# wkentaro/chainer-mask-rcnn

Measured on AMD Instinct MI355X. Metric: images/sec train step, ResNet50-C4 Mask R-CNN, COCO 800x1333, higher is better.
Workload: dtype f32 (bf16x3 split operands, f32 accumulate)

## Files before the change

chainer_mask_rcnn_amd/csrc/conv_gemm.hip:

```cpp
#include <algorithm>
#include <cstring>

#include "conv_gemm_kernel.h"

namespace {

__global__ void splitk_reduce_kernel(const float *__restrict__ ws, int splits, int64_t n,
                                     int64_t stride, float *__restrict__ out)
{
    const int64_t nv = n / 4;
    for (int64_t i = (int64_t)blockIdx.x * blockDim.x + threadIdx.x; i < nv;
         i += (int64_t)gridDim.x * blockDim.x) {
        float4 a = reinterpret_cast<const float4 *>(ws)[i];
        int s = 1;
        for (; s + 4 <= splits; s += 4) {
            const float4 v0 = reinterpret_cast<const float4 *>(ws + (s + 0) * stride)[i];
            const float4 v1 = reinterpret_cast<const float4 *>(ws + (s + 1) * stride)[i];
            const float4 v2 = reinterpret_cast<const float4 *>(ws + (s + 2) * stride)[i];
            const float4 v3 = reinterpret_cast<const float4 *>(ws + (s + 3) * stride)[i];
            a.x += v0.x; a.y += v0.y; a.z += v0.z; a.w += v0.w;
            a.x += v1.x; a.y += v1.y; a.z += v1.z; a.w += v1.w;
            a.x += v2.x; a.y += v2.y; a.z += v2.z; a.w += v2.w;
            a.x += v3.x; a.y += v3.y; a.z += v3.z; a.w += v3.w;
        }
        for (; s < splits; ++s) {
            const float4 v = reinterpret_cast<const float4 *>(ws + s * stride)[i];
            a.x += v.x; a.y += v.y; a.z += v.z; a.w += v.w;
        }
        reinterpret_cast<float4 *>(out)[i] = a;
    }
}

GemmKnobs g_knobs;

inline GemmShape gemm_shape(const GemmParams &p, int mode, bool has_ws)
{
    GemmShape g = {};
    g.mode = mode;
    g.M = p.M; g.N = p.N; g.Kc = p.Kc;
    g.R = p.R; g.S = p.S; g.stride = p.stride; g.pad = p.pad;
    g.gp = p.gp; g.gq = p.gq; g.sh = p.sh; g.sw = p.sw;
    g.ldc = p.ldc; g.out_mode = p.out_mode; g.stem = p.stem; g.perm_n = p.perm_n;
    g.has_ws = has_ws;
    return g;
}

template <int TM, int TN, int MODE>
void launch_kernel(const GemmParams &p, GemmInst inst, int64_t tiles, int splits, hipStream_t s, int batch = 1)
{
    hipEvent_t ev0, ev1;
    mrcnn::prof_take(&ev0, &ev1);
    auto go = [&](auto kernel) {
        hipExtLaunchKernelGGL(kernel, dim3((unsigned)tiles, splits, batch), dim3(256), 0, s, ev0, ev1, 0, p);
    };
    if constexpr (TM == TN && ((MODE == WGRAD && TM == 2) || (MODE == FWD && (TM == 1 || TM == 2)))) {
        if (inst.split) {
            const dim3 grid((unsigned)tiles, splits, batch);
            if (inst.planes == 1) return launch_planes<1>(p, 64 * TM, MODE, inst.variant, grid, s, ev0, ev1);
            if (inst.planes == 2) return launch_planes<2>(p, 64 * TM, MODE, inst.variant, grid, s, ev0, ev1);
            if constexpr (MODE == FWD) {
                if (inst.variant == INST_PW) return go(conv_gemm_kernel<TM, TN, MODE, false, 3, false, true>);
                if (inst.variant == INST_K3) return go(conv_gemm_kernel<TM, TN, MODE, false, 3, false, false, true>);
            }
            return go(conv_gemm_kernel<TM, TN, MODE, false, 3>);
        }
    }
    if constexpr (MODE == WGRAD) {
        if (inst.variant == INST_WPERM) return go(conv_gemm_kernel<TM, TN, MODE, true>);
    }
    go(conv_gemm_kernel<TM, TN, MODE>);
}

template <int TM, int TN, int MODE>
void launch_wino_kernel(const GemmParams &p, const GemmLaunch &l, hipStream_t s)
{
    launch_kernel<TM, TN, MODE>(p, l.inst, l.grid_x, l.grid_y, s, kWinoXi);
}

void launch_w8_kernel(const GemmParams &p, int64_t wgs, int batch, hipStream_t s, int planes = 3)
{
    hipEvent_t ev0, ev1;
    mrcnn::prof_take(&ev0, &ev1);
    const dim3 grid((unsigned)wgs, 1, batch);
    if (planes == 1) return launch_planes<1>(p, kW8BM, FWD, INST_W8, grid, s, ev0, ev1);
    if (planes == 2) return launch_planes<2>(p, kW8BM, FWD, INST_W8, grid, s, ev0, ev1);
    hipExtLaunchKernelGGL((conv_gemm_kernel<2, 2, FWD, false, 3, true>), grid, dim3(512), 0, s, ev0, ev1, 0, p);
}

template <int MODE>
mrcnn::ProfKernelScope gemm_prof(const GemmParams &p, const GemmLaunch &l)
{
    const int small = l.tile >= 128 ? 0 : 1;
    if (MODE == WGRAD)
        return mrcnn::ProfKernelScope(mrcnn::PROF_CONV_WGRAD_128 + small, 2.0 * p.M * p.N * (double)p.Kc,
                                      4.0 * ((double)p.M * p.N + (double)p.Kc * (p.M + (double)p.cin)));
    const int64_t rows = l.m_hi - l.m_lo;
    const double kdepth = (double)p.R * p.S * (p.stem ? 21.0 : (double)p.Kc);
    const double flops = 2.0 * rows * p.N * kdepth;
    const double bytes = 4.0 * ((double)rows * p.N + (double)rows * p.Kc + (double)p.N * kdepth);
    const int kind = l.tile == kW8BM ? mrcnn::PROF_CONV_FWD_W8
                                     : (MODE == FWD ? mrcnn::PROF_CONV_FWD_128 : mrcnn::PROF_CONV_DGRAD_128) + small;
    return mrcnn::ProfKernelScope(kind, flops, bytes);
}

struct FixParams {
    const float *ws;
    float *C;
    const float *bias, *scale, *shift, *residual, *res_g, *res_y, *out_mask_y;
    int splits, rows, N, row0, ldc, flags;
    int perm_n, pq;
    int64_t stride;
};

__global__ void __launch_bounds__(256) splitk_epilogue_kernel(const FixParams f)
{
    const int n4 = f.N / 4;
    const int64_t i = (int64_t)blockIdx.x * blockDim.x + threadIdx.x;
    if (i >= (int64_t)f.rows * n4) return;
    const int r = (int)(i / n4), c = (int)(i - (int64_t)r * n4) * 4;
    float4 a = *reinterpret_cast<const float4 *>(f.ws + (int64_t)r * f.N + c);
    for (int s = 1; s < f.splits; ++s) {
        const float4 v = *reinterpret_cast<const float4 *>(f.ws + s * f.stride + (int64_t)r * f.N + c);
        a.x += v.x; a.y += v.y; a.z += v.z; a.w += v.w;
    }
    float v[4] = {a.x, a.y, a.z, a.w};
    int orow = f.row0 + r;
    if (f.perm_n > 0) {
        const PermRow pr = perm_row(orow, f.pq);
        if (pr.n >= f.perm_n) return;
        orow = pr.n * f.pq + pr.pos;
    }
    const int64_t off = (int64_t)orow * f.ldc + c;
#pragma unroll
    for (int k = 0; k < 4; ++k) {
        float x = v[k];
        if (f.flags & MRCNN_EPI_BIAS) x += f.bias[c + k];
        if (f.flags & MRCNN_EPI_AFFINE) x = x * f.scale[c + k] + (f.shift ? f.shift[c + k] : 0.f);
        if (f.flags & MRCNN_EPI_RESIDUAL) x += f.residual[off + k];
        if (f.flags & MRCNN_EPI_ACCUM) x += f.C[off + k];
        if (f.res_g) x += (!f.res_y || f.res_y[off + k] > 0.f) ? f.res_g[off + k] : 0.f;
        if (f.flags & MRCNN_EPI_RELU) x = fmaxf(x, 0.f);
        if (f.out_mask_y) x = f.out_mask_y[off + k] > 0.f ? x : 0.f;
        v[k] = x;
    }
    *reinterpret_cast<float4 *>(f.C + off) = make_float4(v[0], v[1], v[2], v[3]);
}

template <int MODE>
void slab_sum(const GemmParams &p, int rows_lo, int splits, hipStream_t s)
{
    const int rows = p.M - rows_lo;
    FixParams f = {};
    f.ws = p.split_ws; f.C = p.C;
    f.bias = p.bias; f.scale = p.scale; f.shift = p.shift; f.residual = p.residual;
    f.res_g = p.res_g; f.res_y = p.res_y; f.out_mask_y = p.out_mask_y;
    f.splits = splits; f.rows = rows; f.N = p.N; f.row0 = rows_lo; f.ldc = p.ldc;
    f.flags = p.flags; f.stride = (int64_t)rows * p.N;
    f.perm_n = MODE == FWD ? p.perm_n : 0; f.pq = p.gp * p.gq;
    const int64_t n = (int64_t)rows * (p.N / 4);
    hipLaunchKernelGGL(splitk_epilogue_kernel, dim3((unsigned)mrcnn::ceil_div(n, 256)), dim3(256), 0, s, f);
}

template <int MODE>
int run_plan(const GemmParams &p, const GemmPlan &plan, hipStream_t s)
{
    for (int i = 0; i < plan.n; ++i) {
        const GemmLaunch &l = plan.launch[i];
        GemmParams q = p;
        q.m_lo = l.m_lo;
        q.M = l.m_hi;
        if constexpr (MODE == WGRAD) {
            q.perm_n = plan.perm_n;
            q.split_len = l.split_len;
            q.split_stride = (int64_t)p.M * p.N;
            q.C = plan.sum_splits ? p.split_ws : p.C;
            q.split_ws = nullptr;
        } else if (l.split_len) {
            q.C = p.split_ws;
            q.flags = 0;
            q.bias = q.scale = q.shift = q.residual = q.res_g = q.res_y = q.out_mask_y = nullptr;
            q.split_len = l.split_len;
            q.split_stride = (int64_t)(l.m_hi - l.m_lo) * p.N;
            q.out_row0 = l.m_lo;
            q.c_bytes = (unsigned)(q.split_stride * 4);
        }
        if (l.tail_splits) {
            q.tail_first = l.tail_first;
            q.tail_row0 = l.tail_row0;
            q.tail_splits = l.tail_splits;
            q.tail_split_len = l.tail_split_len;
            q.tail_ws = p.split_ws;
            q.tail_stride = (int64_t)(l.m_hi - l.tail_row0) * p.N;
            q.tail_bytes = (unsigned)(q.tail_stride * 4);
        }
        const auto prof = gemm_prof<MODE>(p, l);
        if (l.tile == kW8BM) {
            if constexpr (MODE == FWD) launch_w8_kernel(q, l.grid_x, 1, s, l.inst.planes);
        } else if (l.tile == 128) {
            launch_kernel<2, 2, MODE>(q, l.inst, l.grid_x, l.grid_y, s);
        } else {
            launch_kernel<1, 1, MODE>(q, l.inst, l.grid_x, l.grid_y, s);
        }
    }
    if constexpr (MODE == WGRAD) {
        if (plan.sum_splits) {
            const int64_t gwsz = (int64_t)p.M * p.N;
            const int64_t blocks = mrcnn::ceil_div(gwsz / 4, 256);
            hipLaunchKernelGGL(splitk_reduce_kernel, dim3((unsigned)blocks), dim3(256), 0, s,
                               (const float *)p.split_ws, plan.sum_splits, gwsz, gwsz, p.C);
        }
        return mrcnn::check_launch("conv_wgrad");
    } else {
        if (plan.sum_splits) slab_sum<MODE>(p, plan.sum_row0, plan.sum_splits, s);
        return mrcnn::check_launch("conv_gemm");
    }
}

template <int MODE>
int launch(const GemmParams &p, hipStream_t s)
{
    return run_plan<MODE>(p, plan_gemm(gemm_shape(p, MODE, p.split_ws != nullptr), g_knobs), s);
}

int check_desc(const mrcnn_conv_desc *d)
{
    MRCNN_REQUIRE(d, "conv: null descriptor");
    MRCNN_REQUIRE(d->N > 0 && d->H > 0 && d->W > 0 && d->C > 0 && d->K > 0 && d->R > 0 && d->S > 0 &&
                      d->stride > 0 && d->pad >= 0,
                  "conv: bad descriptor");
    MRCNN_REQUIRE(d->P == (d->H + 2 * d->pad - d->R) / d->stride + 1 &&
                      d->Q == (d->W + 2 * d->pad - d->S) / d->stride + 1,
                  "conv: output size (%d,%d) inconsistent with input (%d,%d) k=%d s=%d p=%d", d->P,
                  d->Q, d->H, d->W, d->R, d->stride, d->pad);
// ... 514 lines not shown
```

chainer_mask_rcnn_amd/csrc/conv_gemm_kernel.h:

```cpp
#pragma once
#include <type_traits>

#include "common.h"
#include "conv_gemm_plan.h"

namespace {

using namespace mrcnn::gemm;

typedef float f32x16 __attribute__((ext_vector_type(16)));

constexpr int min_blocks(int tm, int mode)
{
    if (!single_buffered(tm, mode)) return 1;
    return tm == 4 ? 2 : (tm == 2 ? 3 : 6);
}
constexpr int KPAD = 4;

constexpr bool is_fwd(int m) { return m == FWD; }

}

namespace mrcnn {
namespace gemm {

struct GemmParams {
    const float *A;
    const float *B;
    float *C;
    const float *bias, *scale, *shift, *residual;
    int M, N;
    int m_lo;
    int Kc;
    int gp, gq;
    int sh, sw;
    int R, S, stride, pad;
    int lda;
    int ldb;
    int ldg;
    int cin;
    int ldc;
    int flags;
    int out_mode;
    int oh, ow, ko;
    int ostride;
    int stem;
    int split_len;
    int64_t split_stride;
    int out_row0;
    int perm_n;
    const float *res_g, *res_y, *out_mask_y;
    float *split_ws;
    unsigned a_bytes, b_bytes, c_bytes;
    int tail_first, tail_splits, tail_split_len, tail_row0;
    unsigned tail_bytes;
    float *tail_ws;
    int64_t tail_stride;
    int64_t batch_a, batch_b, batch_c;
};

struct PermRow { int n, pos; };
__host__ __device__ __forceinline__ PermRow perm_row(int m, int pq)
{
    const int q = m / kPermBlock, img = m - q * kPermBlock;
    const int blk = q / pq;
    PermRow r;
    r.pos = q - blk * pq;
    r.n = blk * kPermBlock + img;
    return r;
}

template <int NP>
void launch_planes(const GemmParams &p, int tile, int mode, int variant, dim3 grid, hipStream_t s, hipEvent_t ev0,
                   hipEvent_t ev1);
extern template void launch_planes<1>(const GemmParams &, int, int, int, dim3, hipStream_t, hipEvent_t, hipEvent_t);
extern template void launch_planes<2>(const GemmParams &, int, int, int, dim3, hipStream_t, hipEvent_t, hipEvent_t);

}
}

namespace {

template <int TM, int TN, int MODE>
struct Cfg {
    static constexpr int BM = 64 * TM, BN = 64 * TN;
    static constexpr bool A_KC = (MODE != WGRAD);
    static constexpr bool B_KC = is_fwd(MODE);
    static constexpr int A_FLOATS = A_KC ? BM * (BK + KPAD) : BK * BM;
    static constexpr int B_FLOATS = B_KC ? BN * (BK + KPAD) : BK * BN;
    static constexpr int A_V4 = BM * BK / 4 / 256;
    static constexpr int B_V4 = BN * BK / 4 / 256;
};

typedef unsigned int u32x4 __attribute__((ext_vector_type(4)));
constexpr unsigned kOOB = 0x80000000u;

__device__ __forceinline__ __amdgpu_buffer_rsrc_t make_rsrc(const void *p, unsigned bytes)
{
    return __builtin_amdgcn_make_buffer_rsrc(const_cast<void *>(p), 0, p ? bytes : 0u, 0x00020000);
}
__device__ __forceinline__ float4 bload4(__amdgpu_buffer_rsrc_t r, unsigned off)
{
    const u32x4 v = __builtin_amdgcn_raw_buffer_load_b128(r, off, 0, 0);
    return make_float4(__uint_as_float(v.x), __uint_as_float(v.y), __uint_as_float(v.z),
                       __uint_as_float(v.w));
}
__device__ __forceinline__ float bload1(__amdgpu_buffer_rsrc_t r, unsigned off)
{
    return __uint_as_float(__builtin_amdgcn_raw_buffer_load_b32(r, off, 0, 0));
}
__device__ __forceinline__ void bstore1(__amdgpu_buffer_rsrc_t r, unsigned off, float v)
{
    __builtin_amdgcn_raw_buffer_store_b32(__float_as_uint(v), r, off, 0, 0);
}
__device__ __forceinline__ void bstore4(__amdgpu_buffer_rsrc_t r, unsigned off, float4 v)
{
    u32x4 u;
    u.x = __float_as_uint(v.x); u.y = __float_as_uint(v.y);
    u.z = __float_as_uint(v.z); u.w = __float_as_uint(v.w);
    __builtin_amdgcn_raw_buffer_store_b128(u, r, off, 0, 0);
}
__device__ __forceinline__ void bstore8(__amdgpu_buffer_rsrc_t r, unsigned off, unsigned a, unsigned b)
{
    typedef unsigned int u32x2 __attribute__((ext_vector_type(2)));
    u32x2 u;
    u.x = a; u.y = b;
    __builtin_amdgcn_raw_buffer_store_b64(u, r, off, 0, 0);
}

typedef __bf16 bf16x2 __attribute__((ext_vector_type(2)));
typedef __bf16 bf16x8 __attribute__((ext_vector_type(8)));
typedef float f32x2 __attribute__((ext_vector_type(2)));
__device__ __forceinline__ unsigned pack_bf16(float a, float b)
{
    const f32x2 v = {a, b};
    return __builtin_bit_cast(unsigned, __builtin_convertvector(v, bf16x2));
}
__device__ __forceinline__ float sub_f32(float a, float b)
{
    float r;
    asm("v_sub_f32 %0, %1, %2" : "=v"(r) : "v"(a), "v"(b));
    return r;
}
template <int NP = 3>
__device__ __forceinline__ void split3(float a, float b, unsigned &h, unsigned &m, unsigned &l)
{
    h = pack_bf16(a, b);
    if constexpr (NP >= 2) {
        a = sub_f32(a, __uint_as_float(h << 16));
        b = sub_f32(b, __uint_as_float(h & 0xffff0000u));
        m = pack_bf16(a, b);
    }
    if constexpr (NP >= 3) {
        a = sub_f32(a, __uint_as_float(m << 16));
        b = sub_f32(b, __uint_as_float(m & 0xffff0000u));
        l = pack_bf16(a, b);
    }
}

template <int G, int NM, int NMD, int ND, int I = 0>
__device__ __forceinline__ void sgb_interleave()
{
    if constexpr (I < G) {
        constexpr int m0 = NM * I / G, m1 = NM * (I + 1) / G;
        constexpr int d0 = m0 >= NMD ? ND : ND * m0 / NMD, d1 = m1 >= NMD ? ND : ND * m1 / NMD;
        if constexpr (m1 > m0) __builtin_amdgcn_sched_group_barrier(0x008, m1 - m0, 0);
        __builtin_amdgcn_sched_group_barrier(0x020, 1, 0);
        if constexpr (d1 > d0) __builtin_amdgcn_sched_group_barrier(0x100, d1 - d0, 0);
        sgb_interleave<G, NM, NMD, ND, I + 1>();
    }
}

template <int TM, int TN, int MODE, bool WPERM = false, int NP = 0, bool W8 = false,
          bool PW = false, bool K3 = false>
__global__ void __launch_bounds__(W8 ? 512 : 256,
                                  NP > 0 ? (TM == 2 ? 2 : 4) : min_blocks(TM, MODE))
conv_gemm_kernel(const GemmParams p)
{
    static_assert(NP >= 0 && NP <= 3, "NP: 0 (fp32 MFMA) or 1 .. 3 bf16 planes");
    constexpr bool SPLIT = NP > 0;
    constexpr int NPROD = NP == 3 ? 6 : NP == 2 ? 3 : 1;
    static_assert(!W8 || (SPLIT && MODE == FWD && TM == 2 && TN == 2),
                  "W8: the split-operand forward form on 64x64 wave tiles");
    static_assert(!WPERM || MODE == WGRAD, "WPERM is a WGRAD-only variant");
    static_assert(!PW || MODE == FWD, "PW: forward form only");
    static_assert(!K3 || (MODE == FWD && !W8 && !PW), "K3: forward form only");
    constexpr bool PWC = W8 || PW;
    constexpr bool GEO = PWC || K3;
    const int gR = PWC ? 1 : K3 ? 3 : p.R, gS = PWC ? 1 : K3 ? 3 : p.S;
    const int gStride = GEO ? 1 : p.stride, gPad = PWC ? 0 : K3 ? 1 : p.pad;
    const int gPermN = GEO ? 0 : p.perm_n;
    const bool gStem = !GEO && p.stem;
    constexpr bool ILV = SPLIT && MODE == FWD;
    static_assert(!SPLIT || (BK == 32 && TM == TN &&
                             ((MODE == FWD && (TM == 1 || TM == 2)) || (MODE == WGRAD && !WPERM && TM == 2))),
                  "SPLIT: forward form (128x128, 64x64) / weight gradient (128x128) only");
    constexpr bool SINGLEBUF = !W8 && (SPLIT || single_buffered(TM, MODE));
    using C_ = Cfg<TM, TN, MODE>;
    constexpr int NT = W8 ? 512 : 256;
    constexpr int BM = (W8 ? 2 : 1) * C_::BM, BN = C_::BN;
    constexpr int AV = BM * BK / 4 / NT, BV = BN * BK / 4 / NT;
    constexpr bool FWDLIKE = is_fwd(MODE);
    constexpr int SROW = MODE == WGRAD ? BK + 8 : BK;
    constexpr int PLA = BM * SROW, PLB = BN * SROW;
    constexpr int STAGE_FLOATS = SPLIT ? 3 * (PLA + PLB) / 2 : C_::A_FLOATS + C_::B_FLOATS;
    __shared__ __attribute__((aligned(16))) float smem_all[1][SINGLEBUF ? 1 : 2][STAGE_FLOATS];

    float (*smem)[STAGE_FLOATS] = smem_all[0];
    constexpr bool WROWPERM = SPLIT && MODE == WGRAD;
    auto swz = [](int row) { return !SPLIT || MODE == WGRAD ? 0 : ((row >> 2) & 3) << 1; };
    const int tid = threadIdx.x;
// ... 254 lines not shown
                const int y = wy_lo + yv, x = wx_lo + pos - yv * wnvx;
                const int a_col = m0 + wa_c4 * 4;
                const int pix_a = y * p.gq + x;
                const int pix_b = (y + wr_u - gPad) * p.sw + x + ws_u - gPad;
#pragma unroll
                for (int i = 0; i < BV; ++i) {
                    const int r = wb_k + B_RPP * i;
                    const int n = blk * BK + r;
                    const bool ok = kb + r < k_end && n < gPermN;
                    const unsigned offa = (unsigned)((n * (p.gp * p.gq) + pix_a) * p.ldg + a_col);
                    ra[i] = bload4(rA, ok && a_col < p.M ? 4u * offa : kOOB);
                    const unsigned offb = (unsigned)((n * (p.sh * p.sw) + pix_b) * p.lda + wc);
                    rb[i] = bload4(rB, ok && wcol_ok ? 4u * offb : kOOB);
                }
                return;
            }
            const unsigned gofs = (unsigned)(kb * p.ldg);
#pragma unroll
            for (int i = 0; i < AV; ++i) {
                const int m = kb + a_krow(i);
                ra[i] = bload4(rA, m < k_end ? 4u * (a_base[i] + gofs) : kOOB);
            }
            if (wpoint) {
                const unsigned xofs = (unsigned)(kb * p.lda);
#pragma unroll
                for (int i = 0; i < BV; ++i) {
                    const int m = kb + b_krow(i);
                    rb[i] = bload4(rB, m < k_end ? 4u * (b_base[i] + xofs) : kOOB);
                }
                return;
            }
#pragma unroll
            for (int i = 0; i < BV; ++i) {
                const int m = kb + b_krow(i);
                const int iy = py[i] * gStride - gPad + wr;
                const int ix = px[i] * gStride - gPad + ws_;
                const bool ok = wcol_ok && m < k_end && (unsigned)iy < (unsigned)p.sh &&
                                (unsigned)ix < (unsigned)p.sw;
                rb[i] = bload4(rB, ok ? 4u * (unsigned)(((pn[i] * p.sh + iy) * p.sw + ix) * p.lda + wc)
                                      : kOOB);
                px[i] += adv_x;
                const int cx = px[i] >= p.gq;
                px[i] -= cx ? p.gq : 0;
                py[i] += adv_y + cx;
                const int cy = py[i] >= p.gp;
                py[i] -= cy ? p.gp : 0;
                pn[i] += adv_n + cy;
            }
        }
    };

    auto store_slice = [&](int buf) {
        if constexpr (SPLIT) {
            unsigned short *pa = reinterpret_cast<unsigned short *>(smem[buf]);
            unsigned short *pb = pa + 3 * PLA;
            auto put = [&](unsigned short *plane0, int plane_len, int row, float4 v) {
                unsigned h0, m0_, l0, h1, m1, l1;
                split3<NP>(v.x, v.y, h0, m0_, l0);
                split3<NP>(v.z, v.w, h1, m1, l1);
                unsigned short *q = plane0 + row * SROW + ((kc_c4 ^ swz(row)) << 2);
                *reinterpret_cast<uint2 *>(q) = make_uint2(h0, h1);
                if constexpr (NP >= 2) *reinterpret_cast<uint2 *>(q + plane_len) = make_uint2(m0_, m1);
                if constexpr (NP >= 3) *reinterpret_cast<uint2 *>(q + 2 * plane_len) = make_uint2(l0, l1);
            };
            if constexpr (MODE == WGRAD) {
                static_assert(AV == 4 && BV == 4, "SPLIT WGRAD: 128x128 tiles");
                auto put_t = [&](unsigned short *plane0, int plane_len, int row0, int kchunk,
                                 const float4 (&r)[4]) {
                    auto e = [&](int i, int c) { return c == 0 ? r[i].x : c == 1 ? r[i].y : c == 2 ? r[i].z : r[i].w; };
#pragma unroll
                    for (int c = 0; c < 4; ++c) {
                        unsigned h0, m0_, l0, h1, m1, l1;
                        split3<NP>(e(0, c), e(1, c), h0, m0_, l0);
                        split3<NP>(e(2, c), e(3, c), h1, m1, l1);
                        const int row = 32 * c + (row0 >> 2);
                        unsigned short *q = plane0 + row * SROW + ((kchunk ^ swz(row)) << 2);
                        *reinterpret_cast<uint2 *>(q) = make_uint2(h0, h1);
                        if constexpr (NP >= 2) *reinterpret_cast<uint2 *>(q + plane_len) = make_uint2(m0_, m1);
                        if constexpr (NP >= 3) *reinterpret_cast<uint2 *>(q + 2 * plane_len) = make_uint2(l0, l1);
                    }
                };
                put_t(pa, PLA, wa_c4 * 4, wa_k, ra);
                put_t(pb, PLB, wb_c4 * 4, wb_k, rb);
                return;
            }
#pragma unroll
            for (int i = 0; i < AV; ++i) {
                put(pa, PLA, kc_row + KC_RPP * i, ra[i]);
            }
#pragma unroll
            for (int i = 0; i < BV; ++i) {
                put(pb, PLB, kc_row + KC_RPP * i, rb[i]);
            }
            return;
        }
        float *sa = smem[buf];
        float *sb = smem[buf] + C_::A_FLOATS;
#pragma unroll
        for (int i = 0; i < AV; ++i) {
            if (C_::A_KC)
                *reinterpret_cast<float4 *>(sa + (kc_row + KC_RPP * i) * (BK + KPAD) + kc_c4 * 4) = ra[i];
            else
                *reinterpret_cast<float4 *>(sa + (wa_k + A_RPP * i) * BM + wa_c4 * 4) = ra[i];
        }
        if (C_::B_KC) {
#pragma unroll
            for (int i = 0; i < BV; ++i)
                *reinterpret_cast<float4 *>(sb + (kc_row + KC_RPP * i) * (BK + KPAD) + kc_c4 * 4) = rb[i];
        } else {
#pragma unroll
            for (int i = 0; i < BV; ++i)
                *reinterpret_cast<float4 *>(sb + (wb_k + B_RPP * i) * BN + wb_c4 * 4) = rb[i];
        }
    };

    f32x16 acc[TM][TN];
#pragma unroll
    for (int i = 0; i < TM; ++i)
#pragma unroll
        for (int j = 0; j < TN; ++j)
#pragma unroll
            for (int e = 0; e < 16; ++e) acc[i][j][e] = 0.f;

    const int li = lane & 31, lk = lane >> 5;

    auto load_frag = [&](const float *sa, const float *sb, int kb, float (&af)[TM][4],
                         float (&bf)[TN][4]) {
#pragma unroll
        for (int i = 0; i < TM; ++i) {
            const int row = wm * (32 * TM) + i * 32 + li;
            if (C_::A_KC) {
                const float4 v = *reinterpret_cast<const float4 *>(
                    sa + row * (BK + KPAD) + kb * 8 + lk * 4);
                af[i][0] = v.x; af[i][1] = v.y; af[i][2] = v.z; af[i][3] = v.w;
            } else {
#pragma unroll
                for (int t = 0; t < 4; ++t) af[i][t] = sa[(kb * 8 + lk * 4 + t) * BM + row];
            }
        }
#pragma unroll
        for (int j = 0; j < TN; ++j) {
            const int col = wn * (32 * TN) + j * 32 + li;
            if (C_::B_KC) {
                const float4 v = *reinterpret_cast<const float4 *>(
                    sb + col * (BK + KPAD) + kb * 8 + lk * 4);
                bf[j][0] = v.x; bf[j][1] = v.y; bf[j][2] = v.z; bf[j][3] = v.w;
            } else {
#pragma unroll
                for (int t = 0; t < 4; ++t) bf[j][t] = sb[(kb * 8 + lk * 4 + t) * BN + col];
            }
        }
    };

    auto compute_ = [&](int buf, auto issue_tag) {
        constexpr bool ISSUE = decltype(issue_tag)::value;
        if constexpr (SPLIT) {
            const unsigned short *pa = reinterpret_cast<const unsigned short *>(smem[buf]);
            const unsigned short *pb = pa + 3 * PLA;
            constexpr int NQ = SPLIT ? NP : 1;
            bf16x8 fa[2][TM][NQ], fb[2][TN][NQ];
            auto frag = [&](int ks, bf16x8 (&a)[TM][NQ], bf16x8 (&b)[TN][NQ]) {
#pragma unroll
                for (int i = 0; i < TM; ++i)
#pragma unroll
                    for (int q = 0; q < NQ; ++q)
                        a[i][q] = *reinterpret_cast<const bf16x8 *>(
                            pa + q * PLA + (wm * (32 * TM) + i * 32 + li) * SROW +
                            (((ks * 4 + lk * 2) ^ swz(wm * (32 * TM) + i * 32 + li)) << 2));
#pragma unroll
                for (int j = 0; j < TN; ++j)
#pragma unroll
                    for (int q = 0; q < NQ; ++q)
                        b[j][q] = *reinterpret_cast<const bf16x8 *>(
                            pb + q * PLB + (wn * (32 * TN) + j * 32 + li) * SROW +
                            (((ks * 4 + lk * 2) ^ swz(wn * (32 * TN) + j * 32 + li)) << 2));
            };
            frag(0, fa[0], fb[0]);
            if constexpr (ISSUE) issue_loads();
#pragma unroll
            for (int ks = 0; ks < BK / 16; ++ks) {
                if (ks + 1 < BK / 16) frag(ks + 1, fa[(ks + 1) & 1], fb[(ks + 1) & 1]);
                constexpr int QA[6] = {0, 2, 1, 1, 0, 0}, QB[6] = {2, 0, 1, 0, 1, 0};
#pragma unroll
                for (int c = 6 - NPROD; c < 6; ++c)
#pragma unroll
                    for (int i = 0; i < TM; ++i)
#pragma unroll
                        for (int j = 0; j < TN; ++j)
                            acc[i][j] = __builtin_amdgcn_mfma_f32_32x32x16_bf16(
                                fa[ks & 1][i][QA[c]], fb[ks & 1][j][QB[c]], acc[i][j], 0, 0, 0);
            }
            if constexpr (ILV && !ISSUE) {
                constexpr int NFR = NQ * (TM + TN), NMH = NPROD * TM * TN;
                __builtin_amdgcn_sched_group_barrier(0x100, NFR, 0);
#pragma unroll
                for (int g = 0; g < NFR; ++g) {
                    __builtin_amdgcn_sched_group_barrier(0x008, 2, 0);
                    __builtin_amdgcn_sched_group_barrier(0x100, 1, 0);
                }
                constexpr int REST = NMH * (BK / 16) - 2 * NFR;
                static_assert(REST >= 0, "two MFMAs per fragment read");
                if constexpr (REST > 0) __builtin_amdgcn_sched_group_barrier(0x008, REST, 0);
            } else if constexpr (ILV) {
                constexpr int NFR = NQ * (TM + TN), NMH = NPROD * TM * TN;
                constexpr int NMD = NMH * (BK / 16 - 1) - 2 * TM * TN > 0 ? NMH * (BK / 16 - 1) - 2 * TM * TN : 1;
                __builtin_amdgcn_sched_group_barrier(0x100, NFR, 0);
                sgb_interleave<NA + NB, NMH * (BK / 16), NMD, NFR>();
            }
            return;
        }
        const float *sa = smem[buf];
        const float *sb = smem[buf] + C_::A_FLOATS;
        float af[2][TM][4], bf[2][TN][4];
        load_frag(sa, sb, 0, af[0], bf[0]);
        constexpr int NR = (C_::A_KC ? TM : 2 * TM) + (C_::B_KC ? TN : 2 * TN);
        constexpr int NMFMA = 4 * TM * TN;
        __builtin_amdgcn_sched_group_barrier(0x100, NR, 0);
#pragma unroll
        for (int kb = 0; kb < BK / 8; ++kb) {
            if (kb + 1 < BK / 8) load_frag(sa, sb, kb + 1, af[(kb + 1) & 1], bf[(kb + 1) & 1]);
#pragma unroll
            for (int t = 0; t < 4; ++t)
#pragma unroll
                for (int i = 0; i < TM; ++i)
#pragma unroll
                    for (int j = 0; j < TN; ++j)
                        acc[i][j] = __builtin_amdgcn_mfma_f32_32x32x2f32(
                            af[kb & 1][i][t], bf[kb & 1][j][t], acc[i][j], 0, 0, 0);
            if (kb + 1 < BK / 8) {
#define MRCNN_SGB_STEP(q)                                         \
    __builtin_amdgcn_sched_group_barrier(0x008, 1, 0);            \
    __builtin_amdgcn_sched_group_barrier(0x100, (NR + 3 - (q)) / 4, 0);
                MRCNN_SGB_STEP(0) MRCNN_SGB_STEP(1) MRCNN_SGB_STEP(2) MRCNN_SGB_STEP(3)
#undef MRCNN_SGB_STEP
                __builtin_amdgcn_sched_group_barrier(0x008, NMFMA - 4, 0);
            } else {
                __builtin_amdgcn_sched_group_barrier(0x008, NMFMA, 0);
            }
        }
    };
    auto compute = [&](int buf) { compute_(buf, std::true_type()); };

    if (nslices > 0) {
        load_slice(0);
        issue_loads();
        store_slice(0);
    }
    if constexpr (W8) {
        auto no_loads = [&]() {
#pragma unroll
            for (int i = 0; i < NA; ++i) oa[i] = kOOB;
#pragma unroll
            for (int i = 0; i < NB; ++i) ob[i] = kOOB;
        };
        if (nslices > 1) {
            load_slice(1);
            issue_loads();
        }
        __syncthreads();
        const bool stage_first = wave >= 4;
        for (int kt = 0; kt < nslices; ++kt) {
            const int cur = kt & 1;
            const bool more = kt + 1 < nslices;
            if (stage_first) {
                if (more) store_slice(cur ^ 1);
                if (kt + 2 < nslices) load_slice(kt + 2); else no_loads();
                compute_(cur, std::true_type());
            } else {
                compute_(cur, std::false_type());
                if (more) store_slice(cur ^ 1);
                if (kt + 2 < nslices) {
                    load_slice(kt + 2);
                    issue_loads();
                }
            }
            __syncthreads();
        }
    } else if (SINGLEBUF) {
        for (int kt = 0; kt < nslices; ++kt) {
            if (kt > 0) {
                __syncthreads();
                store_slice(0);
            }
            __syncthreads();
            if (kt + 1 < nslices) {
                load_slice(kt + 1);
            } else if constexpr (ILV) {
#pragma unroll
                for (int i = 0; i < NA; ++i) oa[i] = kOOB;
#pragma unroll
                for (int i = 0; i < NB; ++i) ob[i] = kOOB;
            }
            compute(0);
        }
    } else {
        __syncthreads();
        for (int kt = 0; kt < nslices; ++kt) {
            const bool more = kt + 1 < nslices;
            if (more) load_slice(kt + 1);
            compute(kt & 1);
            if (more) store_slice((kt + 1) & 1);
            __syncthreads();
        }
    }

    const float *out_base = tail ? p.tail_ws + (int64_t)split * p.tail_stride
                                 : p.C + zb * p.batch_c + (int64_t)split * p.split_stride;
    const __amdgpu_buffer_rsrc_t rC = make_rsrc(out_base, tail ? p.tail_bytes : p.c_bytes);
    const int e_flags = tail ? 0 : p.flags;
    const int e_row0 = tail ? p.tail_row0 : p.out_row0;
    const int e_ldc = tail ? p.N : p.ldc;
    const bool slab_rows = MODE != WGRAD && split_len > 0;
    const __amdgpu_buffer_rsrc_t rRes = make_rsrc(p.residual, p.c_bytes);
    const __amdgpu_buffer_rsrc_t rResG = make_rsrc(p.res_g, p.c_bytes);
    const __amdgpu_buffer_rsrc_t rResY = make_rsrc(p.res_y, p.c_bytes);
    const __amdgpu_buffer_rsrc_t rOutM = make_rsrc(p.out_mask_y, p.c_bytes);
    const bool f_bias = (e_flags & MRCNN_EPI_BIAS) != 0, f_aff = (e_flags & MRCNN_EPI_AFFINE) != 0;
    const bool f_res = (e_flags & MRCNN_EPI_RESIDUAL) != 0, f_relu = (e_flags & MRCNN_EPI_RELU) != 0;
    const bool f_acc = (e_flags & MRCNN_EPI_ACCUM) != 0;
    const bool f_resg = MODE != WGRAD && !tail && p.res_g != nullptr;
    const bool f_resy = f_resg && p.res_y != nullptr;
    const bool f_outm = MODE != WGRAD && !tail && p.out_mask_y != nullptr;
    constexpr int EG = 8;

    if (MODE == FWD && TM >= 2 && (GEO || p.out_mode == OUT_PLAIN)) {
      if constexpr (MODE == FWD && TM >= 2) {
        constexpr int CW = 32 * TN;
        constexpr int LDW = CW + 4;
        constexpr int F4 = CW / 4, RPI = 64 / F4;
        constexpr int NK = 32 / RPI;
        constexpr int QG = TM >= 2 ? 4 : 2;
        __syncthreads();
        float *ep = &smem_all[0][0][0] + wave * (32 * LDW);
        const int c4 = lane % F4, r_in = lane / F4;
        const int col = n0 + wn * CW + c4 * 4;
        const bool col_ok = col < p.N;
        float4 bias4 = make_float4(0.f, 0.f, 0.f, 0.f), scale4 = make_float4(1.f, 1.f, 1.f, 1.f);
        float4 shift4 = bias4;
        if (col_ok) {
            if (f_bias) bias4 = *reinterpret_cast<const float4 *>(p.bias + col);
            if (f_aff) {
                scale4 = *reinterpret_cast<const float4 *>(p.scale + col);
                if (p.shift) shift4 = *reinterpret_cast<const float4 *>(p.shift + col);
            }
        }
        enum { C_BIAS = 1, C_AFF = 2, C_RES = 4, C_RELU = 8, C_ACC = 16, C_RESG = 32, C_RESY = 64,
               C_OUTM = 128 };
        auto run = [&](auto tag) {
            constexpr int F = decltype(tag)::value;
            const bool c_bias = F >= 0 ? (F & C_BIAS) != 0 : f_bias;
            const bool c_aff = F >= 0 ? (F & C_AFF) != 0 : f_aff;
            const bool c_res = F >= 0 ? (F & C_RES) != 0 : f_res;
            const bool c_relu = F >= 0 ? (F & C_RELU) != 0 : f_relu;
            const bool c_acc = F >= 0 ? (F & C_ACC) != 0 : f_acc;
            const bool c_resg = F >= 0 ? (F & C_RESG) != 0 : f_resg;
            const bool c_resy = F >= 0 ? (F & C_RESY) != 0 : f_resy;
            const bool c_outm = F >= 0 ? (F & C_OUTM) != 0 : f_outm;
            const bool natural = F >= 0 || GEO || !(gPermN > 0 && !slab_rows);
#pragma unroll
            for (int i = 0; i < TM; ++i) {
#pragma unroll
                for (int j = 0; j < TN; ++j)
#pragma unroll
                    for (int e = 0; e < 16; ++e)
                        ep[((e & 3) + 8 * (e >> 2) + 4 * lk) * LDW + j * 32 + li] = acc[i][j][e];
                asm volatile("s_waitcnt lgkmcnt(0)" ::: "memory");
#pragma unroll
                for (int kg = 0; kg < NK; kg += QG) {
                    unsigned off[QG];
                    float4 v[QG], a0[QG], a1[QG], a2[QG], a3[QG];
#pragma unroll
                    for (int q = 0; q < QG; ++q) {
                        const int r = (kg + q) * RPI + r_in;
                        v[q] = *reinterpret_cast<const float4 *>(ep + r * LDW + c4 * 4);
                        const int row = m0 + wm * (32 * TM) + i * 32 + r;
                        int orow;
                        if (!natural) {
                            const PermRow pr = perm_row(row < p.M ? row : 0, p.gp * p.gq);
                            orow = pr.n < gPermN ? pr.n * (p.gp * p.gq) + pr.pos : -1;
                        } else {
                            orow = row - e_row0;
                        }
                        const bool ok = col_ok && row < p.M && orow >= 0;
                        off[q] = ok ? 4u * (unsigned)(orow * e_ldc + col) : kOOB;
                    }
                    if (c_res) {
#pragma unroll
                        for (int q = 0; q < QG; ++q) a0[q] = bload4(rRes, off[q]);
                    }
                    if (c_acc) {
#pragma unroll
                        for (int q = 0; q < QG; ++q) a1[q] = bload4(rC, off[q]);
                    }
                    if (c_resg) {
#pragma unroll
                        for (int q = 0; q < QG; ++q) a0[q] = bload4(rResG, off[q]);
                    }
                    if (c_resy) {
#pragma unroll
                        for (int q = 0; q < QG; ++q) a2[q] = bload4(rResY, off[q]);
                    }
                    if (c_outm) {
#pragma unroll
                        for (int q = 0; q < QG; ++q) a3[q] = bload4(rOutM, off[q]);
                    }
#pragma unroll
                    for (int q = 0; q < QG; ++q) {
                        float x[4] = {v[q].x, v[q].y, v[q].z, v[q].w};
                        const float b[4] = {bias4.x, bias4.y, bias4.z, bias4.w};
                        const float sc[4] = {scale4.x, scale4.y, scale4.z, scale4.w};
                        const float sh[4] = {shift4.x, shift4.y, shift4.z, shift4.w};
                        const float r0[4] = {a0[q].x, a0[q].y, a0[q].z, a0[q].w};
                        const float r1[4] = {a1[q].x, a1[q].y, a1[q].z, a1[q].w};
                        const float r2[4] = {a2[q].x, a2[q].y, a2[q].z, a2[q].w};
                        const float r3[4] = {a3[q].x, a3[q].y, a3[q].z, a3[q].w};
#pragma unroll
                        for (int t = 0; t < 4; ++t) {
                            float y = x[t];
                            if (c_bias) y += b[t];
                            if (c_aff) y = y * sc[t] + sh[t];
                            if (c_res) y += r0[t];
                            if (c_acc) y += r1[t];
                            if (c_resy) y += r2[t] > 0.f ? r0[t] : 0.f;
                            else if (c_resg) y += r0[t];
                            if (c_relu) y = fmaxf(y, 0.f);
                            if (c_outm) y = r3[t] > 0.f ? y : 0.f;
                            x[t] = y;
                        }
                        bstore4(rC, off[q], make_float4(x[0], x[1], x[2], x[3]));
                    }
                }
            }
        };
        const int combo = (f_bias ? C_BIAS : 0) | (f_aff ? C_AFF : 0) | (f_res ? C_RES : 0) |
                          (f_relu ? C_RELU : 0) | (f_acc ? C_ACC : 0) | (f_resg ? C_RESG : 0) |
                          (f_resy ? C_RESY : 0) | (f_outm ? C_OUTM : 0);
        const bool permuted = !GEO && gPermN > 0 && !slab_rows;
#define MRCNN_EPI_CASE(F) case (F): run(std::integral_constant<int, (F)>()); break;
        switch (permuted ? -1 : combo) {
            MRCNN_EPI_CASE(0)
            MRCNN_EPI_CASE(C_AFF)
            MRCNN_EPI_CASE(C_AFF | C_RELU)
            MRCNN_EPI_CASE(C_AFF | C_RES | C_RELU)
            MRCNN_EPI_CASE(C_BIAS)
            MRCNN_EPI_CASE(C_BIAS | C_RELU)
            MRCNN_EPI_CASE(C_AFF | C_OUTM)
            MRCNN_EPI_CASE(C_RESG | C_OUTM)
            MRCNN_EPI_CASE(C_RESG)
            MRCNN_EPI_CASE(C_ACC | C_OUTM)
            MRCNN_EPI_CASE(C_ACC)
        default: run(std::integral_constant<int, -1>()); break;
        }
#undef MRCNN_EPI_CASE
        return;
      }
    }
    if constexpr (WROWPERM) {
        static_assert(TM == 2 && TN == 2, "SPLIT WGRAD: 128x128 tiles");
        const int col = n0 + 4 * li + 2 * wn;
        const bool col_ok = col < p.N;
#pragma unroll
        for (int i = 0; i < TM; ++i) {
#pragma unroll
            for (int g = 0; g < 16 / EG; ++g) {
                unsigned off[EG];
                float row_scale[EG];
#pragma unroll
                for (int q = 0; q < EG; ++q) {
                    const int e = g * EG + q;
                    const int row = m0 + 4 * ((e & 3) + 8 * (e >> 2) + 4 * lk) + 2 * wm + i;
                    off[q] = (col_ok && row < p.M) ? 4u * (unsigned)(row * e_ldc + col) : kOOB;
                    row_scale[q] = (p.scale && row < p.M) ? p.scale[row] : 1.f;
                }
#pragma unroll
                for (int q = 0; q < EG; ++q) {
                    const float v0 = acc[i][0][g * EG + q] * row_scale[q];
                    const float v1 = acc[i][1][g * EG + q] * row_scale[q];
                    bstore8(rC, off[q], __float_as_uint(v0), __float_as_uint(v1));
                }
            }
        }
        return;
    }
#pragma unroll
    for (int j = 0; j < TN; ++j) {
        const int col = n0 + wn * (32 * TN) + j * 32 + li;
        const bool col_ok = col < p.N;
        const int colc = col_ok ? col : 0;
        float bias = 0.f, scale = 1.f, shift = 0.f;
        if (MODE != WGRAD) {
            if (f_bias) bias = p.bias[!GEO && p.out_mode == OUT_DECONV ? colc % p.ko : colc];
            if (f_aff) { scale = p.scale[colc]; shift = p.shift ? p.shift[colc] : 0.f; }
        }
        int col_off = colc;
        if (MODE != WGRAD && !GEO && p.out_mode == OUT_DECONV) {
            const int ab = colc / p.ko, o = colc - ab * p.ko;
            col_off = ((ab >> 1) * (2 * p.gq) + (ab & 1)) * p.ko + o;
        }
#pragma unroll
        for (int i = 0; i < TM; ++i) {
#pragma unroll
            for (int g = 0; g < 16 / EG; ++g) {
                unsigned off[EG];
#pragma unroll
                for (int q = 0; q < EG; ++q) {
                    const int e = g * EG + q;
                    const int row = m0 + wm * (32 * TM) + i * 32 + (e & 3) + 8 * (e >> 2) + 4 * lk;
                    int o;
                    if (MODE != WGRAD && !GEO && p.out_mode != OUT_PLAIN) {
                        const int rr = row < p.M ? row : 0;
                        const int n = rr / (p.gp * p.gq);
                        const int rem = rr - n * (p.gp * p.gq);
                        const int gy = rem / p.gq, gx = rem - gy * p.gq;
                        if (p.out_mode == OUT_STRIDED)
                            o = ((n * p.oh + gy * (p.ostride ? p.ostride : gStride)) * p.ow +
                                 gx * (p.ostride ? p.ostride : gStride)) * p.ldc + col_off;
                        else
                            o = ((n * (2 * p.gp) + 2 * gy) * (2 * p.gq) + 2 * gx) * p.ko + col_off;
                    } else if (FWDLIKE && !GEO && gPermN > 0 && !slab_rows) {
                        const PermRow pr = perm_row(row < p.M ? row : 0, p.gp * p.gq);
                        o = pr.n < gPermN ? (pr.n * (p.gp * p.gq) + pr.pos) * p.ldc + col_off : -1;
                    } else {
                        o = (row - e_row0) * e_ldc + col_off;
                    }
                    off[q] = (col_ok && row < p.M && o >= 0) ? 4u * (unsigned)o : kOOB;
                }
                float aux0[EG], aux1[EG], aux2[EG], aux3[EG];
                if (MODE != WGRAD) {
                    if (f_res) {
#pragma unroll
                        for (int q = 0; q < EG; ++q) aux0[q] = bload1(rRes, off[q]);
                    }
                    if (f_acc) {
#pragma unroll
                        for (int q = 0; q < EG; ++q) aux1[q] = bload1(rC, off[q]);
                    }
                    if (f_resg) {
#pragma unroll
                        for (int q = 0; q < EG; ++q) aux0[q] = bload1(rResG, off[q]);
                    }
                    if (f_resy) {
#pragma unroll
                        for (int q = 0; q < EG; ++q) aux2[q] = bload1(rResY, off[q]);
                    }
                    if (f_outm) {
#pragma unroll
                        for (int q = 0; q < EG; ++q) aux3[q] = bload1(rOutM, off[q]);
                    }
                }
                float row_scale[EG];
                if (MODE == WGRAD && p.scale) {
#pragma unroll
                    for (int q = 0; q < EG; ++q) {
                        const int e = g * EG + q;
                        const int row = m0 + wm * (32 * TM) + i * 32 + (e & 3) + 8 * (e >> 2) + 4 * lk;
                        row_scale[q] = row < p.M ? p.scale[row] : 0.f;
                    }
// ... 25 lines not shown
```

chainer_mask_rcnn_amd/csrc/conv_gemm_plan.h:

```cpp
#pragma once
#include <algorithm>
#include <cstdint>
#include <cstring>

namespace mrcnn {
namespace gemm {

constexpr int BK = 32;
enum Mode { FWD = 0, DGRAD = 1, WGRAD = 2 };
enum OutMode { OUT_PLAIN = 0, OUT_STRIDED = 1, OUT_DECONV = 2 };
constexpr int64_t kSlotsBig = 512, kSlotsSmall = 1024;
constexpr int64_t kSplitWsBytes = 192ll << 20;
constexpr int kPermBlock = 128;
constexpr int kW8BM = 256, kW8BN = 128;

inline int64_t cdiv(int64_t a, int64_t b) { return (a + b - 1) / b; }

constexpr bool single_buffered(int tm, int mode)
{
    if (tm == 1) return mode == 0;
    return tm >= 2 && (mode == 0 || mode == 2);
}

struct GemmKnobs {
    int split_bf16 = 3;
    int split_planes = 3;
    int big_split_k = -1;
    int big_split_min_slices = 16;
    int w8 = 1, w8_min_k = 256;
    int pw = 3;
    int fused_tail = 512;
    int big_min_tiles = 384;
    int small_m_split = 0;
    int tiny_split = 1;
    int position_major_rows = 1;
};

inline bool knob_value_ok(const char *name, int value)
{
    return strcmp(name, "split_planes") != 0 || (value >= 1 && value <= 3);
}

inline bool set_knob(GemmKnobs &k, const char *name, int value)
{
    const struct { const char *name; int *at; } table[] = {
        {"split_bf16", &k.split_bf16}, {"split_planes", &k.split_planes}, {"big_split_k", &k.big_split_k},
        {"big_split_min_slices", &k.big_split_min_slices}, {"w8_min_k", &k.w8_min_k}, {"w8", &k.w8},
        {"pw", &k.pw}, {"fused_tail", &k.fused_tail}, {"big_min_tiles", &k.big_min_tiles},
        {"small_m_split", &k.small_m_split}, {"tiny_split", &k.tiny_split},
        {"position_major_rows", &k.position_major_rows}};
    for (const auto &t : table) {
        if (strcmp(name, t.name) != 0) continue;
        if (t.at == &k.fused_tail) value = value == 1 ? 512 : value;
        if (t.at == &k.position_major_rows) value = value != 0;
        *t.at = value;
        return true;
    }
    return false;
}

struct GemmShape {
    int mode;
    int M, N, Kc;
    int R, S, stride, pad;
    int gp, gq, sh, sw;
    int ldc, out_mode, stem, perm_n;
    bool has_ws;
    int64_t pixels;
    int n_img, C;
};

inline int choose_perm(const GemmKnobs &k, int n_img, int gp, int gq, int R, int S, int stride, int pad_eff)
{
    if (!k.position_major_rows || R * S <= 1 || R * S > 16 || stride != 1 || pad_eff <= 0) return 0;
    if (gp * gq > 256 || n_img < 64) return 0;
    return n_img;
}

inline bool pw_plain(const GemmShape &p)
{
    return p.R == 1 && p.S == 1 && p.stride == 1 && p.pad == 0 && p.perm_n == 0 && !p.stem && p.gp == p.sh &&
           p.gq == p.sw && p.out_mode == OUT_PLAIN;
}

inline bool k3_plain(const GemmShape &p)
{
    return p.R == 3 && p.S == 3 && p.stride == 1 && p.pad == 1 && p.perm_n == 0 && !p.stem &&
           p.out_mode == OUT_PLAIN;
}

inline bool w8_ok(const GemmShape &p, const GemmKnobs &k, int batch = 1)
{
    if (!k.w8 || !(k.split_bf16 & 1) || !pw_plain(p)) return false;
    const int64_t tm = cdiv(p.M, kW8BM), tn = cdiv(p.N, kW8BN);
    return p.N >= kW8BN && p.Kc >= k.w8_min_k && tm * tn * batch >= 768 && (p.M % kW8BM == 0 || p.M >= 16 * kW8BM);
}

enum Variant { INST_GENERAL = 0, INST_PW, INST_K3, INST_WPERM, INST_W8 };
struct GemmInst {
    bool split;
    int variant;
    int planes;
};

inline GemmInst pick_inst(const GemmShape &p, int tm, const GemmKnobs &k)
{
    if (p.mode == WGRAD) {
        if (tm == 2 && (k.split_bf16 & 1) && p.perm_n == 0) return {true, INST_GENERAL, k.split_planes};
        return {false, p.perm_n > 0 ? INST_WPERM : INST_GENERAL, 0};
    }
    if (p.mode == FWD && (k.split_bf16 & (tm == 2 ? 1 : 2))) {
        if ((k.pw & 1) && pw_plain(p)) return {true, INST_PW, k.split_planes};
        if ((k.pw & 2) && k3_plain(p)) return {true, INST_K3, k.split_planes};
        return {true, INST_GENERAL, k.split_planes};
    }
    return {false, INST_GENERAL, 0};
}

struct GemmLaunch {
    int tile;
    int m_lo, m_hi;
    int64_t grid_x;
    int grid_y;
    int split_len;
    int tail_first, tail_row0, tail_splits, tail_split_len;
    GemmInst inst;
};

struct GemmPlan {
    const char *label;
    int n;
    GemmLaunch launch[2];
    int sum_row0, sum_splits;
    int64_t k_extent;
    int perm_n;
};

inline bool can_split_rows(const GemmShape &p)
{
    return p.has_ws && p.mode != WGRAD && p.out_mode == OUT_PLAIN && !p.stem && p.N % 4 == 0 &&
           p.ldc == p.N;
}

inline int64_t fit_ws(int64_t splits, int64_t rows, int N)
{
    while (splits > 1 && rows * N * splits * 4 > kSplitWsBytes) --splits;
    return splits;
}

inline int64_t k_splits(int total_slices, int depth_div, int64_t target_wgs, int64_t tiles, int64_t rows, int N,
                        int64_t cap)
{
    return fit_ws(std::min<int64_t>(std::min<int64_t>(cap, total_slices / depth_div), cdiv(target_wgs, tiles)),
                  rows, N);
}

inline int total_slices(const GemmShape &p) { return p.R * p.S * (int)cdiv(p.Kc, BK); }

inline GemmLaunch *add_tiles(GemmPlan &g, const GemmShape &p, int tm, int m_lo, int m_hi, const GemmKnobs &k)
{
    const int64_t blocks = cdiv(m_hi - m_lo, 64 * tm) * cdiv(p.N, 64 * tm);
    if (blocks <= 0) return nullptr;
    GemmLaunch &l = g.launch[g.n++];
    l.tile = 64 * tm;
    l.m_lo = m_lo;
    l.m_hi = m_hi;
    l.grid_x = blocks;
    l.grid_y = 1;
    l.inst = pick_inst(p, tm, k);
    return &l;
}

inline void add_split_rows(GemmPlan &g, const GemmShape &p, int tm, int rows_lo, int splits, const GemmKnobs &k)
{
    GemmLaunch *l = add_tiles(g, p, tm, rows_lo, p.M, k);
    if (!l) return;
    l->split_len = (int)cdiv(total_slices(p), splits);
    l->grid_y = (int)cdiv(total_slices(p), l->split_len);
    g.sum_row0 = rows_lo;
    g.sum_splits = l->grid_y;
}

inline void set_tail(GemmPlan &g, GemmLaunch &l, int rows_main, int64_t tail_first, int64_t tail_tiles,
                     int slices, int64_t splits)
{
    l.tail_split_len = (int)cdiv(slices, splits);
    l.tail_splits = (int)cdiv(slices, l.tail_split_len);
    l.tail_first = (int)tail_first;
    l.tail_row0 = rows_main;
    l.grid_x = l.tail_first + tail_tiles * l.tail_splits;
    g.sum_row0 = rows_main;
    g.sum_splits = l.tail_splits;
}

inline bool add_fused_tail(GemmPlan &g, const GemmShape &p, int tm, int rows_main, const GemmKnobs &k)
{
    const int BM = 64 * tm;
    if (!k.fused_tail || !can_split_rows(p) || rows_main <= 0 || rows_main % BM != 0 || rows_main >= p.M)
        return false;
    const int64_t ntn = cdiv(p.N, BM);
    const int64_t main_tiles = (rows_main / BM) * ntn;
    const int64_t tail_tiles = cdiv(p.M - rows_main, BM) * ntn;
    const int64_t splits = k_splits(total_slices(p), 4, k.fused_tail, tail_tiles, p.M - rows_main, p.N, 16);
    if (splits < 2) return false;
    set_tail(g, *add_tiles(g, p, tm, 0, p.M, k), rows_main, main_tiles, tail_tiles, total_slices(p), splits);
    return true;
}
// ... 239 lines not shown
```

Measured before the change: 87.24.

## Prefetch epilogue residual/accumulate operands during final K-slices of conv GEMM

Adds an epilogue prefetch path for split-bf16 forward conv GEMM kernels. During the last one or two K-slice iterations it issues buffer loads of the first epilogue operand (residual, grouped residual, accumulate target or output mask) into registers, interleaved with the MFMA compute. It also prefetches the next row-block while the current block is staged through shared memory. The aim is to hide global-memory latency for fused epilogue reads. The cost is higher register pressure, which may lower occupancy, and a more complex slice loop with peeled final iterations. It is enabled by default through a new knob.

```diff
diff --git a/chainer_mask_rcnn_amd/csrc/conv_gemm.hip b/chainer_mask_rcnn_amd/csrc/conv_gemm.hip
--- a/chainer_mask_rcnn_amd/csrc/conv_gemm.hip
+++ b/chainer_mask_rcnn_amd/csrc/conv_gemm.hip
@@ -46,8 +46,10 @@
 }
 
 template <int TM, int TN, int MODE>
-void launch_kernel(const GemmParams &p, GemmInst inst, int64_t tiles, int splits, hipStream_t s, int batch = 1)
-{
+void launch_kernel(const GemmParams &p0, GemmInst inst, int64_t tiles, int splits, hipStream_t s, int batch = 1)
+{
+    GemmParams p = p0;
+    p.epi_prefetch = g_knobs.epi_prefetch;
     hipEvent_t ev0, ev1;
     mrcnn::prof_take(&ev0, &ev1);
     auto go = [&](auto kernel) {
@@ -77,8 +79,10 @@
     launch_kernel<TM, TN, MODE>(p, l.inst, l.grid_x, l.grid_y, s, kWinoXi);
 }
 
-void launch_w8_kernel(const GemmParams &p, int64_t wgs, int batch, hipStream_t s, int planes = 3)
-{
+void launch_w8_kernel(const GemmParams &p0, int64_t wgs, int batch, hipStream_t s, int planes = 3)
+{
+    GemmParams p = p0;
+    p.epi_prefetch = g_knobs.epi_prefetch;
     hipEvent_t ev0, ev1;
     mrcnn::prof_take(&ev0, &ev1);
     const dim3 grid((unsigned)wgs, 1, batch);
diff --git a/chainer_mask_rcnn_amd/csrc/conv_gemm_kernel.h b/chainer_mask_rcnn_amd/csrc/conv_gemm_kernel.h
--- a/chainer_mask_rcnn_amd/csrc/conv_gemm_kernel.h
+++ b/chainer_mask_rcnn_amd/csrc/conv_gemm_kernel.h
@@ -57,6 +57,7 @@
     float *tail_ws;
     int64_t tail_stride;
     int64_t batch_a, batch_b, batch_c;
+    int epi_prefetch;
 };
 
 struct PermRow { int n, pos; };
@@ -617,8 +618,8 @@
         }
     };
 
-    auto compute_ = [&](int buf, auto issue_tag) {
-        constexpr bool ISSUE = decltype(issue_tag)::value;
+    auto compute_ = [&](int buf, auto issue) {
+        constexpr bool ISSUE = !std::is_same<decltype(issue), std::false_type>::value;
         if constexpr (SPLIT) {
             const unsigned short *pa = reinterpret_cast<const unsigned short *>(smem[buf]);
             const unsigned short *pb = pa + 3 * PLA;
@@ -641,7 +642,7 @@
                             (((ks * 4 + lk * 2) ^ swz(wn * (32 * TN) + j * 32 + li)) << 2));
             };
             frag(0, fa[0], fb[0]);
-            if constexpr (ISSUE) issue_loads();
+            if constexpr (ISSUE) issue();
 #pragma unroll
             for (int ks = 0; ks < BK / 16; ++ks) {
                 if (ks + 1 < BK / 16) frag(ks + 1, fa[(ks + 1) & 1], fb[(ks + 1) & 1]);
@@ -704,7 +705,42 @@
             }
         }
     };
-    auto compute = [&](int buf) { compute_(buf, std::true_type()); };
+    auto compute = [&](int buf) { compute_(buf, issue_loads); };
+
+    constexpr int CW = 32 * TN;
+    constexpr int F4 = CW / 4, RPI = 64 / F4;
+    constexpr int NK = 32 / RPI;
+    constexpr bool EPF = SPLIT && MODE == FWD && TM >= 2 && GEO;
+    constexpr int PF_PART = W8 ? NK / 2 : NK;
+    const int e_c4 = lane % F4, e_rin = lane / F4;
+    const int e_col = n0 + wn * CW + e_c4 * 4;
+    const float *pf_ptr = nullptr;
+    if constexpr (EPF) {
+        if (p.epi_prefetch && !tail && split_len == 0 && nslices > 0)
+            pf_ptr = (p.flags & MRCNN_EPI_RESIDUAL) ? p.residual
+                     : p.res_g                      ? p.res_g
+                     : (p.flags & MRCNN_EPI_ACCUM)  ? p.C + zb * p.batch_c
+                                                    : p.out_mask_y;
+    }
+    const bool pf = pf_ptr != nullptr;
+    const __amdgpu_buffer_rsrc_t rFirst = make_rsrc(pf_ptr, p.c_bytes);
+    float4 fo[TM][NK];
+    const int pf_row0 = m0 + wm * (32 * TM) + e_rin;
+    const unsigned pf_base = 4u * (unsigned)((pf_row0 - p.out_row0) * p.ldc + e_col);
+    auto pf_off = [&](int i, int pass) {
+        const int r = i * 32 + pass * RPI;
+        const bool ok = (e_col < p.N) & (pf_row0 + r < p.M) & (pf_row0 + r >= p.out_row0);
+        return ok ? pf_base + 4u * (unsigned)(r * p.ldc) : kOOB;
+    };
+    auto pf_issue = [&](auto part) {
+        constexpr int T0 = decltype(part)::value * PF_PART;
+#pragma unroll
+        for (int t = T0; t < T0 + PF_PART; ++t) fo[0][t] = bload4(rFirst, pf_off(0, t));
+    };
+    auto pf_part0 = [&]() { pf_issue(std::integral_constant<int, 0>()); };
+    auto pf_part1 = [&]() {
+        if constexpr (W8) pf_issue(std::integral_constant<int, 1>());
+    };
 
     if (nslices > 0) {
         load_slice(0);
@@ -724,40 +760,70 @@
         }
         __syncthreads();
         const bool stage_first = wave >= 4;
-        for (int kt = 0; kt < nslices; ++kt) {
+        auto w8_slice = [&](int kt, auto pm) {
+            constexpr int PM = decltype(pm)::value;
             const int cur = kt & 1;
             const bool more = kt + 1 < nslices;
             if (stage_first) {
                 if (more) store_slice(cur ^ 1);
-                if (kt + 2 < nslices) load_slice(kt + 2); else no_loads();
-                compute_(cur, std::true_type());
+                if constexpr (PM == 0) {
+                    if (kt + 2 < nslices) load_slice(kt + 2); else no_loads();
+                    compute_(cur, issue_loads);
+                } else if constexpr (PM == 1) {
+                    compute_(cur, pf_part0);
+                } else {
+                    compute_(cur, pf_part1);
+                }
             } else {
                 compute_(cur, std::false_type());
                 if (more) store_slice(cur ^ 1);
-                if (kt + 2 < nslices) {
-                    load_slice(kt + 2);
-                    issue_loads();
+                if constexpr (PM == 0) {
+                    if (kt + 2 < nslices) {
+                        load_slice(kt + 2);
+                        issue_loads();
+                    }
+                } else if constexpr (PM == 1) {
+                    pf_part0();
+                    pf_part1();
                 }
             }
             __syncthreads();
+        };
+        const int nloop = pf ? max(nslices - 2, 0) : nslices;
+        for (int kt = 0; kt < nloop; ++kt) w8_slice(kt, std::integral_constant<int, 0>());
+        if (pf) {
+            if (nslices >= 2) {
+                w8_slice(nslices - 2, std::integral_constant<int, 1>());
+            } else {
+                pf_part0();
+                if (!stage_first) pf_part1();
+            }
+            w8_slice(nslices - 1, std::integral_constant<int, 2>());
         }
     } else if (SINGLEBUF) {
-        for (int kt = 0; kt < nslices; ++kt) {
+        auto sb_slice = [&](int kt, auto pm) {
             if (kt > 0) {
                 __syncthreads();
                 store_slice(0);
             }
             __syncthreads();
-            if (kt + 1 < nslices) {
-                load_slice(kt + 1);
-            } else if constexpr (ILV) {
-#pragma unroll
-                for (int i = 0; i < NA; ++i) oa[i] = kOOB;
-#pragma unroll
-                for (int i = 0; i < NB; ++i) ob[i] = kOOB;
-            }
-            compute(0);
-        }
+            if constexpr (decltype(pm)::value) {
+                compute_(0, pf_part0);
+            } else {
+                if (kt + 1 < nslices) {
+                    load_slice(kt + 1);
+                } else if constexpr (ILV) {
+#pragma unroll
+                    for (int i = 0; i < NA; ++i) oa[i] = kOOB;
+#pragma unroll
+                    for (int i = 0; i < NB; ++i) ob[i] = kOOB;
+                }
+                compute(0);
+            }
+        };
+        const int nloop = pf ? nslices - 1 : nslices;
+        for (int kt = 0; kt < nloop; ++kt) sb_slice(kt, std::false_type());
+        if (pf) sb_slice(nslices - 1, std::true_type());
     } else {
         __syncthreads();
         for (int kt = 0; kt < nslices; ++kt) {
@@ -790,15 +856,12 @@
 
     if (MODE == FWD && TM >= 2 && (GEO || p.out_mode == OUT_PLAIN)) {
       if constexpr (MODE == FWD && TM >= 2) {
-        constexpr int CW = 32 * TN;
         constexpr int LDW = CW + 4;
-        constexpr int F4 = CW / 4, RPI = 64 / F4;
-        constexpr int NK = 32 / RPI;
         constexpr int QG = TM >= 2 ? 4 : 2;
         __syncthreads();
         float *ep = &smem_all[0][0][0] + wave * (32 * LDW);
-        const int c4 = lane % F4, r_in = lane / F4;
-        const int col = n0 + wn * CW + c4 * 4;
+        const int c4 = e_c4, r_in = e_rin;
+        const int col = e_col;
         const bool col_ok = col < p.N;
         float4 bias4 = make_float4(0.f, 0.f, 0.f, 0.f), scale4 = make_float4(1.f, 1.f, 1.f, 1.f);
         float4 shift4 = bias4;
@@ -821,6 +884,9 @@
             const bool c_resg = F >= 0 ? (F & C_RESG) != 0 : f_resg;
             const bool c_resy = F >= 0 ? (F & C_RESY) != 0 : f_resy;
             const bool c_outm = F >= 0 ? (F & C_OUTM) != 0 : f_outm;
+            const bool pre_res = pf && c_res, pre_resg = pf && !c_res && c_resg;
+            const bool pre_acc = pf && !c_res && !c_resg && c_acc;
+            const bool pre_outm = pf && !c_res && !c_resg && !c_acc && c_outm;
             const bool natural = F >= 0 || GEO || !(gPermN > 0 && !slab_rows);
 #pragma unroll
             for (int i = 0; i < TM; ++i) {
@@ -830,6 +896,12 @@
                     for (int e = 0; e < 16; ++e)
                         ep[((e & 3) + 8 * (e >> 2) + 4 * lk) * LDW + j * 32 + li] = acc[i][j][e];
                 asm volatile("s_waitcnt lgkmcnt(0)" ::: "memory");
+                if constexpr (EPF) {
+                    if (pf && i + 1 < TM) {
+#pragma unroll
+                        for (int t = 0; t < NK; ++t) fo[i + 1 < TM ? i + 1 : i][t] = bload4(rFirst, pf_off(i + 1, t));
+                    }
+                }
 #pragma unroll
                 for (int kg = 0; kg < NK; kg += QG) {
                     unsigned off[QG];
@@ -850,24 +922,44 @@
                         off[q] = ok ? 4u * (unsigned)(orow * e_ldc + col) : kOOB;
                     }
                     if (c_res) {
-#pragma unroll
-                        for (int q = 0; q < QG; ++q) a0[q] = bload4(rRes, off[q]);
+                        if (pre_res) {
+#pragma unroll
+                            for (int q = 0; q < QG; ++q) a0[q] = fo[i][kg + q];
+                        } else {
+#pragma unroll
+                            for (int q = 0; q < QG; ++q) a0[q] = bload4(rRes, off[q]);
+                        }
                     }
                     if (c_acc) {
-#pragma unroll
-                        for (int q = 0; q < QG; ++q) a1[q] = bload4(rC, off[q]);
+                        if (pre_acc) {
+#pragma unroll
+                            for (int q = 0; q < QG; ++q) a1[q] = fo[i][kg + q];
+                        } else {
+#pragma unroll
+                            for (int q = 0; q < QG; ++q) a1[q] = bload4(rC, off[q]);
+                        }
                     }
                     if (c_resg) {
-#pragma unroll
-                        for (int q = 0; q < QG; ++q) a0[q] = bload4(rResG, off[q]);
+                        if (pre_resg) {
+#pragma unroll
+                            for (int q = 0; q < QG; ++q) a0[q] = fo[i][kg + q];
+                        } else {
+#pragma unroll
+                            for (int q = 0; q < QG; ++q) a0[q] = bload4(rResG, off[q]);
+                        }
                     }
                     if (c_resy) {
 #pragma unroll
                         for (int q = 0; q < QG; ++q) a2[q] = bload4(rResY, off[q]);
                     }
                     if (c_outm) {
-#pragma unroll
-                        for (int q = 0; q < QG; ++q) a3[q] = bload4(rOutM, off[q]);
+                        if (pre_outm) {
+#pragma unroll
+                            for (int q = 0; q < QG; ++q) a3[q] = fo[i][kg + q];
+                        } else {
+#pragma unroll
+                            for (int q = 0; q < QG; ++q) a3[q] = bload4(rOutM, off[q]);
+                        }
                     }
 #pragma unroll
                     for (int q = 0; q < QG; ++q) {
diff --git a/chainer_mask_rcnn_amd/csrc/conv_gemm_plan.h b/chainer_mask_rcnn_amd/csrc/conv_gemm_plan.h
--- a/chainer_mask_rcnn_amd/csrc/conv_gemm_plan.h
+++ b/chainer_mask_rcnn_amd/csrc/conv_gemm_plan.h
@@ -34,6 +34,7 @@
     int small_m_split = 0;
     int tiny_split = 1;
     int position_major_rows = 1;
+    int epi_prefetch = 1;
 };
 
 inline bool knob_value_ok(const char *name, int value)
@@ -48,11 +49,11 @@
         {"big_split_min_slices", &k.big_split_min_slices}, {"w8_min_k", &k.w8_min_k}, {"w8", &k.w8},
         {"pw", &k.pw}, {"fused_tail", &k.fused_tail}, {"big_min_tiles", &k.big_min_tiles},
         {"small_m_split", &k.small_m_split}, {"tiny_split", &k.tiny_split},
-        {"position_major_rows", &k.position_major_rows}};
+        {"position_major_rows", &k.position_major_rows}, {"epi_prefetch", &k.epi_prefetch}};
     for (const auto &t : table) {
         if (strcmp(name, t.name) != 0) continue;
         if (t.at == &k.fused_tail) value = value == 1 ? 512 : value;
-        if (t.at == &k.position_major_rows) value = value != 0;
+        if (t.at == &k.position_major_rows || t.at == &k.epi_prefetch) value = value != 0;
         *t.at = value;
         return true;
     }
```

New measurement: 87.38, median of 6. About the same (+0.2%).
